# yahoo0742/COSNet

Hardware: AMD Instinct MI355X
Metric: frame-pairs/sec (fwd+bwd) at 473x473 RGBD (higher is better)
Workload: dtype bf16; 1 GPU; RGBDSegmentation_RAA train step (fwd+loss+bwd+SGD), 473x473, batch 4 pairs/GPU; model=RGBDSegmentation_RAA(Bottleneck,[3,4,23,3],[3,4,6,3],1), global_batch=4, parallelism=dp1

## Files before the change

### cosnet_amd/_native.py

```python
import ctypes
import os

import torch

_HERE = os.path.dirname(os.path.abspath(__file__))
LIB_PATH = os.environ.get("COSNET_HIP_LIB") or os.path.join(_HERE, "_lib", "libcosnet_hip.so")

DT_F32 = 0
DT_BF16 = 1

_P = ctypes.c_void_p
_I = ctypes.c_int
_L = ctypes.c_longlong
_F = ctypes.c_float
_S = ctypes.c_size_t

_SIGS = {
    "cn_conv_fwd": (_I, [_I, _P, _L, _I, _I, _I, _I, _P, _I, _I, _I, _I, _I, _I, _P, _P, _L, _I, _I, _P]),
    "cn_conv_fwd_ws": (_I, [_I, _P, _L, _I, _I, _I, _I, _P, _I, _I, _I, _I, _I, _I, _P, _P, _L, _I, _I,
                            _P, _S, _P]),
    "cn_conv_fwd_workspace_floats": (_S, [_I, _I, _I, _I]),
    "cn_conv_dgrad": (_I, [_I, _P, _L, _I, _I, _I, _I, _P, _I, _I, _I, _I, _I, _I, _P, _L, _I, _I, _I, _P]),
    "cn_conv_wgrad_workspace_floats": (_S, [_I, _I, _I, _I, _I, _I, _I, _I]),
    "cn_conv_wgrad": (_I, [_I, _P, _L, _I, _I, _I, _I, _P, _L, _I, _I, _I, _I, _I, _I, _I, _I, _P, _P, _P]),
    "cn_conv_wgrad_grouped": (_I, [_I, _I, _P, _L, _I, _I, _I, _I, _P, _L, _I, _I, _I, _I, _I, _I, _I, _I,
                                   _P, _P]),
    "cn_conv_wgrad_grouped_workspace_floats": (_S, [_I, _I, _I, _I, _I, _I, _I, _I, _I]),
    "cn_conv_wgrad_grouped_ws": (_I, [_I, _I, _P, _L, _I, _I, _I, _I, _P, _L, _I, _I, _I, _I, _I, _I, _I,
                                      _I, _P, _P, _S, _P]),
    "cn_splitk_reduce": (_I, [_P, _I, _L, _L, _P, _I, _P]),
    "cn_fp8_quant": (_I, [_I, _P, _L, _I, _I, _P, _L, _P, _I, _P]),
    "cn_fp8_quant_fmt": (_I, [_I, _I, _P, _L, _I, _I, _P, _L, _P, _I, _P]),
    "cn_conv_dgrad_fp8": (_I, [_P, _L, _I, _I, _I, _I, _P, _I, _I, _I, _I, _I, _P, _L, _I, _I, _I,
                               _P, _P, _P]),
    "cn_fp8_update": (_I, [_P, _I, _F, _P]),
    "cn_fp8_quant_multi": (_I, [_P, _I, _P]),
    "cn_conv_fwd_fp8": (_I, [_P, _L, _I, _I, _I, _I, _P, _I, _I, _I, _I, _I, _I, _P, _P, _L, _I, _I, _P,
                             _P, _P]),
    "cn_conv_fwd_bn_workspace_floats": (_S, [_I, _I, _I, _I]),
    "cn_conv_fwd_bn_grouped": (_I, [_I, _P, _L, _I, _I, _I, _I, _I, _P, _I, _I, _I, _P, _P, _P, _L, _I,
                                    _P, _P, _P, _P, _P, _F, _F, _P]),
    "cn_conv_fwd_fp8_bn": (_I, [_P, _L, _I, _I, _I, _I, _P, _I, _I, _I, _I, _I, _I, _P, _P, _L, _I, _I,
                                _P, _P, _I, _P, _P, _P, _P, _P, _F, _F, _P]),
    "cn_conv_fwd_bn": (_I, [_I, _P, _L, _I, _I, _I, _I, _P, _I, _I, _I, _I, _I, _I, _P, _P, _L, _I, _I,
                            _I, _P, _P, _P, _P, _P, _F, _F, _P]),
    "cn_conv_dgrad_bn_workspace_floats": (_S, [_I, _I, _I, _I]),
    "cn_conv_dgrad_bn": (_I, [_I, _P, _L, _I, _I, _I, _I, _P, _I, _I, _I, _I, _I, _P, _L, _I, _I, _P,
                              _L, _P, _P, _P, _P, _P, _P, _P, _P]),
    "cn_bn_bwd_apply": (_I, [_I, _P, _L, _P, _L, _I, _I, _P, _P, _P, _P, _P, _P, _P, _L, _P]),
    "cn_gemm": (_I, [_I, _I, _I, _I, _I, _I, _I, _I, _P, _L, _L, _P, _L, _L, _P, _L, _L, _I, _I, _F, _P, _I, _I, _L, _P]),
    "cn_bn_workspace_floats": (_S, [_I, _I, _I, _I]),
    "cn_bn_stats": (_I, [_I, _P, _L, _I, _I, _I, _P, _P, _P, _P, _F, _F, _P, _P]),
    "cn_bn_eval_params": (_I, [_P, _P, _I, _F, _P, _P, _P]),
    "cn_bn_apply": (_I, [_I, _P, _L, _I, _I, _I, _P, _P, _P, _P, _P, _L, _P, _L, _P, _P, _P, _P, _I, _P, _P, _L, _P]),
    "cn_bn_apply_fp8": (_I, [_I, _P, _L, _I, _I, _I, _P, _P, _P, _P, _P, _L, _P, _L, _P, _P, _P, _P, _I, _P,
                             _P, _L, _P, _L, _P, _P]),
    "cn_bn_apply_ex": (_I, [_I, _P, _L, _I, _I, _I, _P, _P, _P, _P, _P, _L, _P, _L, _P, _P, _P, _P, _I, _P,
                            _P, _L, _P, _L, _P, _P, _L, _P]),
    "cn_bn_set_tuning": (_I, [_I, _I]),
    "cn_bn_bwd": (_I, [_I, _P, _L, _P, _L, _P, _L, _I, _I, _P, _P, _P, _P, _I, _P, _P, _P, _P, _P, _L, _P, _L, _P, _P]),
    "cn_coatt_workspace_floats": (_S, [_I, _I, _I]),
    "cn_coatt_softmax": (_I, [_I, _P, _I, _I, _I, _P, _P, _P, _P]),
    "cn_coatt_dscore": (_I, [_I, _P, _P, _P, _P, _P, _P, _I, _I, _I, _P, _P]),
    "cn_coatt_fused_fwd": (_I, [_P, _L, _P, _L, _P, _L, _I, _I, _I, _P, _P, _L, _P]),
    "cn_coatt_fused_fwd_ws": (_I, [_P, _L, _P, _L, _P, _L, _I, _I, _I, _P, _P, _L, _P, _S, _P]),
    "cn_coatt_fused_workspace_bytes": (_S, [_I, _I, _I]),
    "cn_coatt_f8_workspace_bytes": (_S, [_I, _I]),
    "cn_coatt_f8_fwd": (_I, [_P, _L, _P, _L, _P, _L, _I, _I, _I, _P, _P, _L, _P, _P, _P, _S, _P]),
    "cn_coatt_f8_train_workspace_bytes": (_S, [_I, _I]),
    "cn_coatt_f8_train_fwd": (_I, [_P, _L, _P, _L, _P, _L, _I, _I, _I, _P, _P, _L, _P, _P, _P, _P, _P, _L, _P, _S, _P]),
    "cn_coatt_flash_fwd": (_I, [_P, _L, _P, _L, _P, _L, _I, _I, _I, _P, _P, _L, _P, _P, _P]),
    "cn_coatt_flash_fwd_ws": (_I, [_P, _L, _P, _L, _P, _L, _I, _I, _I, _P, _P, _L, _P, _P, _P, _S, _P]),
    "cn_coatt_flash_pv": (_I, [_P, _L, _P, _L, _P, _L, _P, _I, _I, _I, _P, _L, _I, _P]),
    "cn_coatt_flash_dvat": (_I, [_P, _L, _P, _L, _P, _L, _P, _L, _P, _L, _P, _P, _P, _P, _I, _I, _I, _P,
                                 _L, _I, _P]),
    "cn_coatt_flash_dvat_ws": (_I, [_P, _L, _P, _L, _P, _L, _P, _L, _P, _L, _P, _P, _P, _P, _I, _I, _I, _P,
                                    _L, _I, _P, _S, _P]),
    "cn_coatt_flash_bwd_workspace_bytes": (_S, [_I, _I]),
    "cn_coatt_flash_pv_ws": (_I, [_P, _L, _P, _L, _P, _L, _P, _I, _I, _I, _P, _L, _I, _P, _S, _P]),
    "cn_rowdot_seg": (_I, [_I, _P, _L, _P, _L, _I, _I, _I, _I, _P, _P]),
    "cn_nchw_to_nhwc": (_I, [_I, _P, _I, _I, _I, _I, _I, _P, _P]),
    "cn_weight_prep": (_I, [_I, _P, _I, _I, _I, _I, _P, _P, _P]),
    "cn_maxpool_fwd": (_I, [_I, _P, _I, _I, _I, _I, _I, _I, _I, _I, _I, _P, _P, _P]),
    "cn_maxpool_bwd": (_I, [_I, _P, _P, _I, _I, _I, _I, _I, _I, _I, _I, _I, _P, _P]),
    "cn_avgpool": (_I, [_I, _P, _L, _I, _I, _I, _F, _P, _P, _P]),
    "cn_avgpool_workspace_floats": (_S, [_I, _I, _I, _I]),
    "cn_bcast_rows": (_I, [_I, _P, _I, _I, _I, _F, _P, _L, _I, _P]),
    "cn_gate_fwd": (_I, [_I, _P, _L, _I, _I, _P, _P, _P, _L, _P, _P]),
    "cn_gate_bwd": (_I, [_I, _P, _L, _P, _L, _P, _I, _I, _P, _I, _P, _L, _P, _P, _P, _P]),
    "cn_colpart_workspace_floats": (_S, [_I, _I]),
    "cn_mean_rows": (_I, [_P, _I, _I, _P, _P]),
    "cn_sum_rows": (_I, [_P, _I, _I, _P, _P]),
    "cn_scale_dev": (_I, [_P, _L, _P, _P, _P]),
    "cn_scale": (_I, [_P, _L, _F, _P]),
    "cn_soft_iou": (_I, [_P, _P, _I, _L, _P, _P, _P, _P]),
    "cn_frame_resize": (_I, [_I, _P, _I, _L, _L, _L, _I, _I, _I, _I, _P, _P, _I, _I, _I, _I, _P]),
    "cn_gemm_force_config": (_I, [_I]),
    "cn_gemm_set_wgrad_target": (_I, [_I]),
    "cn_coatt_force_variant": (_I, [_I]),
    "cn_head_fwd": (_I, [_I, _P, _L, _P, _L, _I, _I, _I, _P, _P, _P, _L, _P, _P]),
    "cn_head_bwd": (_I, [_I, _P, _L, _P, _I, _I, _I, _P, _P, _L, _P, _P, _P, _P]),
    "cn_upsample_sigmoid": (_I, [_P, _I, _I, _I, _I, _I, _I, _P, _P]),
    "cn_upsample_sigmoid_bwd": (_I, [_P, _P, _I, _I, _I, _I, _I, _I, _P, _P]),
    "cn_count_ge": (_I, [_P, _L, _F, _P, _P]),
    "cn_loss_workspace_floats": (_S, [_L]),
    "cn_bce_l1": (_I, [_P, _P, _L, _F, _F, _P, _P, _P, _P]),
    "cn_bce_l1_devcount": (_I, [_P, _P, _L, _P, ctypes.c_double, _F, _P, _P, _P, _P]),
    "cn_sgd": (_I, [_P, _I, _P, _F, _F, _P]),
    "cn_rowdot": (_I, [_I, _P, _L, _P, _L, _I, _I, _P, _P]),
    "cn_colsum": (_I, [_I, _P, _L, _I, _I, _P, _P, _P]),
    "cn_cast2d": (_I, [_I, _I, _P, _L, _I, _I, _P, _L, _I, _P]),
    "cn_build_source_hash": (ctypes.c_char_p, []),
    "cn_build_experimental": (_I, []),
    "cn_conv_wgrad_fp8_workspace_floats": (_S, [_I, _I, _I, _I, _I, _I, _I, _I]),
    "cn_conv_wgrad_fp8": (_I, [_I, _P, _L, _I, _I, _I, _I, _P, _L, _I, _I, _I, _I, _I, _I, _I, _I,
                               _P, _P, _P, _P, _S, _P]),
}

_lib = None


class NativeError(RuntimeError):
    pass


def load():
    global _lib
    if _lib is not None:
        return _lib
    if not os.path.exists(LIB_PATH):
        raise NativeError("libcosnet_hip.so not built (%s); run __graft_entry__.build()" % LIB_PATH)
    lib = ctypes.CDLL(LIB_PATH, mode=ctypes.RTLD_GLOBAL)
    for name, (res, args) in _SIGS.items():
        if os.environ.get("COSNET_HIP_LIB") and not hasattr(lib, name):
            continue
        fn = getattr(lib, name)
        fn.restype = res
        fn.argtypes = args
    _lib = lib
    return lib


HASHED_SOURCES = ["gemm.hip", "conv.hip", "bn.hip", "ew.hip", "coatt.hip", "coatt_fused.hip",
                  "coatt_q48.hip", "coatt_flash.hip", "coatt_f8.hip", "fp8.hip", "frames.hip", "eval.hip",
                  "common.h", "gemm.h", "coatt_fused.h", "../../include/cosnet_hip.h"]


def source_hash():
    import hashlib
    h = hashlib.sha256()
    for f in HASHED_SOURCES:
        with open(os.path.join(_HERE, "csrc", f), "rb") as fh:
            h.update(fh.read())
    return h.hexdigest()[:16]


def build_info():
    import hashlib
    lib_hash = load().cn_build_source_hash().decode()
    with open(LIB_PATH, "rb") as fh:
        so = hashlib.sha256(fh.read()).hexdigest()[:16]
    src = source_hash()
    return {"lib_source_hash": lib_hash, "tree_source_hash": src, "built_from_tree": lib_hash == src,
            "lib_sha256": so, "lib": os.path.relpath(LIB_PATH, os.path.dirname(_HERE))}


def exported_symbols():
    return sorted(_SIGS.keys())


_ERR = {-1: "shape", -2: "alignment", -3: "unsupported", -4: "hip runtime"}


def call(name, *args):
    rc = getattr(load(), name)(*args)
    if rc != 0:
        raise NativeError("%s failed: %s (%d)" % (name, _ERR.get(rc, "hipError"), rc))
    return rc


def query(name, *args):
    return getattr(load(), name)(*args)


def stream():
    return torch.cuda.current_stream().cuda_stream


def ptr(t):
    return None if t is None else t.data_ptr()


def dtype_code(dt):
    if dt == torch.bfloat16:
        return DT_BF16
    if dt == torch.float32:
        return DT_F32
    raise NativeError("unsupported compute dtype %s" % dt)
```

### cosnet_amd/csrc/gemm.h

```cpp
#pragma once
#include "common.h"

enum LoadKind { L_KC_DENSE = 0, L_KC_CONV = 1, L_MC_DENSE = 2, L_MC_CONV = 3,
                L_KC_CONV_G = 4 };

struct ConvGeom {
  int N, H, W, C;
  int OH, OW;
  int KH, KW;
  int st;
  int off_y, off_x, step_y, step_x;
  FastDiv div_C, div_KW, div_OW, div_OHW;
};

constexpr int GEMM_MAXG = 24;
struct GemmGroup {
  const void* A[GEMM_MAXG];
  const void* B[GEMM_MAXG];
  void* C[GEMM_MAXG];
  const float* SA[GEMM_MAXG];
  const float* SB[GEMM_MAXG];
  const float* bias[GEMM_MAXG];
  float* ST[GEMM_MAXG];
  int dil[GEMM_MAXG];
};

struct GemmArgs {
  int M, N, K;
  int ka_lim, kb_lim;
  const void* A; long long lda, a_bs;
  const void* B; long long ldb, b_bs;
  void* C; long long ldc, c_bs;
  const float* bias;
  ConvGeom ga, gb;
  int k_chunk, nsplit;
  int row_map;
  FastDiv rm_div_OW, rm_div_OHW;
  int rm_H, rm_W;
  int c_mode;
  long long slab;
  float alpha;
  const float* scale_a;
  const float* scale_b;
  int cfg;
  int st_mode;
  float* st_ws;
  long long st_plane;
  int st_seg_rows;
  const void* br_x; long long br_ldx;
  const float* br_mean; const float* br_invstd; const float* br_gamma; const float* br_beta;
  int ngroup;
  GemmGroup grp;
  int wt;
};

int cn_gemm_dispatch(const GemmArgs& a, int dtype, int c_f32, int la, int lb, int batch, hipStream_t st);
int cn_gemm_pick(int M, int N, int K, int batch_splits);
long long cn_gemm_cfg_blocks(int cfg, int M, int N);
int cn_gemm_bm(int dtype, int M, int N, int K, int cfg_or_minus1);
int cn_splitk_reduce_impl(const float* ws, int nsplit, long long slab, long long n, float* out,
                          int accumulate, hipStream_t st);
```

### cosnet_amd/csrc/gemm.hip

```cpp
#include "common.h"
#include "gemm.h"
#include "../../include/cosnet_hip.h"

#include <cstdlib>
#include <type_traits>

namespace {

template <class T> struct Frag;
template <> struct Frag<bf16> { typedef bf16x8 type; };
template <> struct Frag<float> { typedef f32x4 type; };

__device__ __forceinline__ int mc_swz(int k, int granules_per_row) {
  int h = (k & 3) | (((k >> 3) & 1) << 2);
  return (granules_per_row >= 32 ? h : (h & 3)) << 2;
}

__device__ __forceinline__ int mc_swz8(int k) { return (k & 7) ^ ((k >> 5) & 1); }

__device__ __attribute__((aligned(16))) unsigned g_zero16[4];

__device__ __forceinline__ void glds16(const void* src, char* lds_wave_base) {
  __builtin_amdgcn_global_load_lds((const __attribute__((address_space(1))) void*)src,
                                   (__attribute__((address_space(3))) void*)lds_wave_base, 16, 0, 0);
}

constexpr unsigned BUF_OOB = 0x80000000u;
__device__ __forceinline__ __amdgpu_buffer_rsrc_t buf_rsrc(const void* base) {
  return __builtin_amdgcn_make_buffer_rsrc(const_cast<void*>(base), 0, (int)BUF_OOB, 0x00020000);
}
__device__ __forceinline__ void blds16(__amdgpu_buffer_rsrc_t r, unsigned voff, unsigned soff,
                                       char* lds_wave_base) {
  __builtin_amdgcn_raw_ptr_buffer_load_lds(r, (__attribute__((address_space(3))) void*)lds_wave_base,
                                           16, (int)voff, (int)soff, 0, 0);
}

template <class T, int ROWS, int KIND, int NT> struct Loader {
  static constexpr int VEC = VecOf<T>::N;
  static constexpr int BK = 8 * VEC;
  static constexpr int NCH = ROWS * 8 / NT;
  static constexpr int RSTEP = NT / 8;
  static_assert(NCH >= 1 && NCH * NT == ROWS * 8, "tile rows must fill whole chunk rounds");
  static constexpr bool MC = (KIND == L_MC_DENSE || KIND == L_MC_CONV);
  static constexpr bool BUF = (KIND == L_KC_DENSE || KIND == L_KC_CONV || KIND == L_MC_DENSE);
  static constexpr int CPR = ROWS / VEC;
  static constexpr int KROW_STEP = NT / CPR;
  static constexpr int RB = ROWS * (int)sizeof(T);
  static constexpr unsigned SZ = sizeof(T);
  static_assert(!(MC && sizeof(T) == 1) || CPR == 8, "fp8 MC tiles are 128 columns wide (mc_swz8)");

  long long ld;
  int klim;
  int kbeg;
  int kcol;
  bool ok[NCH];
  __amdgpu_buffer_rsrc_t rsrc;
  unsigned voff[NCH];
  int img[NCH], by[NCH], bx[NCH];
  int ctap;
  const T* base;
  const T* ptr[NCH];
  int ry[NCH], sx[NCH], cic[NCH];
  int pim[NCH], poy[NCH], pox[NCH], pp[NCH];
  int ax, ay, aim;
  ConvGeom g;

  __device__ __forceinline__ void init(const T* b, long long ld_, int lim, int klim_,
                                       const ConvGeom& geo, int origin, int tid, int kbeg_) {
    ld = ld_; klim = klim_; kbeg = kbeg_;
    base = b;
    if (!MC) {
      const int pos = tid & 7;
      kcol = (pos ^ ((tid >> 3) & 7)) * VEC;
      if (KIND == L_KC_DENSE) rsrc = buf_rsrc(b + (long long)origin * ld);
      if (KIND == L_KC_CONV) rsrc = buf_rsrc(b);
#pragma unroll
      for (int i = 0; i < NCH; ++i) {
        const int rl = (tid >> 3) + RSTEP * i;
        const int row = origin + rl;
        ok[i] = row < lim;
        const int rr = ok[i] ? row : 0;
        if (KIND == L_KC_DENSE) {
          voff[i] = ok[i] ? (unsigned)((rl * ld + kcol) * SZ) : BUF_OOB;
        } else {
          int q, rem, oy, ox;
          fdivmod(rr, geo.div_OHW, q, rem);
          fdivmod(rem, geo.div_OW, oy, ox);
          img[i] = ok[i] ? q : -1;
          by[i] = oy * geo.st + geo.off_y;
          bx[i] = ox * geo.st + geo.off_x;
        }
      }
      if (KIND == L_KC_CONV || KIND == L_KC_CONV_G) {
        g = geo;
        ctap = -1;
      }
    } else {
      const int pos = tid % CPR;
      if (KIND == L_MC_DENSE) rsrc = buf_rsrc(b + (long long)kbeg_ * ld + origin);
#pragma unroll
      for (int i = 0; i < NCH; ++i) {
        const int krl = tid / CPR + KROW_STEP * i;
        const int cchunk = (sizeof(T) == 2) ? (pos ^ (mc_swz(krl, RB / 8) >> 1))
                         : (sizeof(T) == 1) ? (pos ^ mc_swz8(krl)) : pos;
        const int col = origin + cchunk * VEC;
        ok[i] = col < lim;
        if (KIND == L_MC_DENSE) {
          voff[i] = ok[i] ? (unsigned)((krl * ld + cchunk * VEC) * SZ) : BUF_OOB;
        } else {
          const int nn = ok[i] ? col : 0;
          int tap, r, s2;
          fdivmod(nn, geo.div_C, tap, cic[i]);
          fdivmod(tap, geo.div_KW, r, s2);
          ry[i] = r * geo.step_y + geo.off_y;
          sx[i] = s2 * geo.step_x + geo.off_x;
          pp[i] = kbeg_ + krl;
          int q, rem, oy, ox;
// ... 104 lines not shown
    }
  }
};

template <int ROWS, bool MC>
__device__ __forceinline__ bf16x8 read_frag_bf16(const char* lds, int rowbase, int p, int lane) {
  int g = lane >> 4;
  if (!MC) {
    int row = rowbase + (lane & 15);
    int c = 4 * p + g;
    return *(const bf16x8*)(lds + row * 128 + ((c ^ (row & 7)) << 4));
  } else {
    constexpr int RB = ROWS * 2;
    int q = (lane & 15) >> 2, pp = lane & 3;
    int gm = (rowbase >> 2) + pp;
    int k1 = 32 * p + 8 * g + q, k2 = k1 + 4;
    const char* a1 = lds + k1 * RB + ((gm ^ mc_swz(k1, RB / 8)) << 3);
    const char* a2 = lds + k2 * RB + ((gm ^ mc_swz(k2, RB / 8)) << 3);
    s16x4 lo = __builtin_amdgcn_ds_read_tr16_b64_v4i16(LDS_PTR(s16x4, a1));
    s16x4 hi = __builtin_amdgcn_ds_read_tr16_b64_v4i16(LDS_PTR(s16x4, a2));
    typedef __attribute__((ext_vector_type(8))) short s16x8;
    s16x8 r = __builtin_shufflevector(lo, hi, 0, 1, 2, 3, 4, 5, 6, 7);
    return __builtin_bit_cast(bf16x8, r);
  }
}

__device__ __forceinline__ i32x8 read_frag_f8(const char* lds, int rowbase, int lane) {
  const int row = rowbase + (lane & 15), g = lane >> 4;
  const u32x4 lo = *(const u32x4*)(lds + row * 128 + (((2 * g) ^ (row & 7)) << 4));
  const u32x4 hi = *(const u32x4*)(lds + row * 128 + (((2 * g + 1) ^ (row & 7)) << 4));
  i32x8 r;
  r[0] = lo.x; r[1] = lo.y; r[2] = lo.z; r[3] = lo.w; r[4] = hi.x; r[5] = hi.y; r[6] = hi.z; r[7] = hi.w;
  return r;
}

typedef __attribute__((ext_vector_type(2))) int i32x2;
__device__ __forceinline__ i32x8 read_frag_f8_mc(const char* lds, int colbase, int lane) {
  const int i = lane & 15, g = lane >> 4, q = i >> 1, pp = i & 1;
  const int cb = colbase >> 4;
  i32x8 r;
#pragma unroll
  for (int j = 0; j < 4; ++j) {
    const int k = 32 * g + 8 * j + q;
    const char* a = lds + k * 128 + ((cb ^ mc_swz8(k)) << 4) + 8 * pp;
    const i32x2 v = __builtin_amdgcn_ds_read_tr8_b64_v2i32(LDS_PTR(i32x2, a));
    r[2 * j] = v.x;
    r[2 * j + 1] = v.y;
  }
  return r;
}

template <int ROWS>
__device__ __forceinline__ f32x4 read_frag_f32_kc(const char* lds, int rowbase, int p, int lane) {
  int row = rowbase + (lane & 15);
  int c = 4 * p + (lane >> 4);
  return *(const f32x4*)(lds + row * 128 + ((c ^ (row & 7)) << 4));
}
template <int ROWS>
__device__ __forceinline__ float read_frag_f32_mc(const char* lds, int rowbase, int p, int j, int lane) {
  int k = 16 * p + 4 * (lane >> 4) + j;
  int col = rowbase + (lane & 15);
  return *(const float*)(lds + k * (ROWS * 4) + col * 4);
}

template <class CT> __device__ __forceinline__ void store_c(CT* c, float v, int mode);
template <> __device__ __forceinline__ void store_c<float>(float* c, float v, int mode) {
  if (mode == 1) atomicAdd(c, v);
  else if (mode == 2) *c += v;
  else *c = v;
}
template <> __device__ __forceinline__ void store_c<bf16>(bf16* c, float v, int mode) {
  if (mode == 2) v += (float)*c;
  *c = (bf16)v;
}

}

template <int G>
__device__ __forceinline__ void wait_tiles(int n) {
  if (n <= 0) asm volatile("s_waitcnt vmcnt(0)" ::: "memory");
  else if (n == 1) asm volatile("s_waitcnt vmcnt(%0)" :: "n"(G) : "memory");
  else if (n == 2) asm volatile("s_waitcnt vmcnt(%0)" :: "n"(2 * G) : "memory");
  else asm volatile("s_waitcnt vmcnt(%0)" :: "n"(3 * G) : "memory");
}

__device__ __forceinline__ void raw_barrier() {
  asm volatile("" ::: "memory");
  __builtin_amdgcn_s_barrier();
  asm volatile("" ::: "memory");
}

#ifndef CN_GEMM_GROUP_M
#define CN_GEMM_GROUP_M 8
#endif
#ifndef CN_GEMM_PRIO
#define CN_GEMM_PRIO 0
#endif
#ifndef CN_GEMM_ZREMAP
#define CN_GEMM_ZREMAP 1
#endif

template <class T, class CT, int BM, int BN, int WM, int WN, int S, int LA, int LB, int EPI = 0, int PP = 0>
__global__ __launch_bounds__(WM * WN * 64 * (PP == 2 ? 2 : 1), (EPI && sizeof(T) == 2 && BM * BN <= 128 * 128 && S == 2) ? 4 : 1) void gemm_kernel(GemmArgs p) {
  constexpr bool KSG = PP == 2;
  constexpr int NT = WM * WN * 64 * (KSG ? 2 : 1);
  constexpr int VEC = VecOf<T>::N;
  constexpr int BK = 8 * VEC;
  constexpr int ABYTES = BM * 128, BBYTES = BN * 128;
  constexpr int STAGE = ABYTES + BBYTES;
  constexpr int TM = BM / WM, TN = BN / WN;
  constexpr int RM = TM / 16, RN = TN / 16;
  constexpr bool AMC = (LA == L_MC_DENSE || LA == L_MC_CONV);
  constexpr bool BMC = (LB == L_MC_DENSE || LB == L_MC_CONV);
  typedef Loader<T, BM, LA, NT> LdA;
  typedef Loader<T, BN, LB, NT> LdB;
  constexpr int G = LdA::NCH + LdB::NCH;
  static_assert(S >= 2 && S <= 4, "2..4 stages");
  __shared__ __attribute__((aligned(16))) char smem[S * STAGE];

  const int tid = threadIdx.x, lane = tid & 63, wave = tid >> 6;
  const int kg = KSG ? wave / (WM * WN) : 0;
  const int wl = KSG ? wave % (WM * WN) : wave;
  const int wm = wl / WN, wn = wl % WN;
  static_assert(!KSG || (sizeof(T) == 2 && !AMC && !BMC), "KSG: bf16 k-contiguous operands");
  int tm, tn, bz;
  {
    const int nwg = gridDim.x * gridDim.y;
#if CN_GEMM_ZREMAP
    const int all = nwg * gridDim.z;
    const int orig = blockIdx.x + blockIdx.y * gridDim.x + blockIdx.z * nwg;
#else
    const int all = nwg;
    const int orig = blockIdx.x + blockIdx.y * gridDim.x;
#endif
    int glin = orig;
    if (all >= 16) {
      const int xcd = orig & 7, q = all >> 3, r = all & 7;
      glin = (xcd < r ? xcd * (q + 1) : r * (q + 1) + (xcd - r) * q) + (orig >> 3);
    }
#if CN_GEMM_ZREMAP
    bz = glin / nwg;
#else
    bz = blockIdx.z;
#endif
    const int lin = glin - (glin / nwg) * nwg;
#if CN_GEMM_GROUP_M > 0
    {
      const int gm = CN_GEMM_GROUP_M;
      const int per = gm * gridDim.y;
      const int grp = lin / per, first = grp * gm;
      const int gsz = min((int)gridDim.x - first, gm);
      const int r = lin - grp * per;
      tm = first + r % gsz;
      tn = r / gsz;
    }
#else
    tm = lin % gridDim.x;
    tn = lin / gridDim.x;
#endif
  }
  const int m0 = tm * BM, n0 = tn * BN;
  const int batch = bz / p.nsplit, split = bz - batch * p.nsplit;
  int kbeg = split * p.k_chunk;
  int kend = min(p.K, kbeg + p.k_chunk);
  ConvGeom gA = p.ga;
  if constexpr (LA == L_KC_CONV) {
    if (p.ngroup && p.grp.dil[batch] > 0) {
      const int dl = p.grp.dil[batch];
      gA.off_y = gA.off_x = -dl;
      gA.step_y = gA.step_x = dl;
    }
  }
// ... 653 lines not shown
          const int c = pick_cfg(a, batch);
          if (c == 18) return launch_c<T, CT, 18, LA, LB>(a, batch, st);
          if (c == 19) return launch_c<T, CT, 19, LA, LB>(a, batch, st);
          return launch_c<T, CT, 20, LA, LB>(a, batch, st);
        } else {
          if (pick_cfg(a, batch) == 20) return launch_c<T, CT, 10, LA, LB>(a, batch, st);
          return launch_c<T, CT, 11, LA, LB>(a, batch, st);
        }
      }
      default: return launch_c<T, CT, 12, LA, LB>(a, batch, st);
    }
  }
}

template <class T, class CT>
static int launch_conv_g(const GemmArgs& a, int batch, hipStream_t st) {
  if constexpr (sizeof(T) == 4) {
    if (a.N <= 64 || cfg_blocks(1, a, batch) < 384) return launch_c<T, CT, 0, L_KC_CONV_G, L_KC_DENSE>(a, batch, st);
    return launch_c<T, CT, 1, L_KC_CONV_G, L_KC_DENSE>(a, batch, st);
  } else {
    const int c = pick_cfg(a, batch);
    if (c == 12) return launch_c<T, CT, 12, L_KC_CONV_G, L_KC_DENSE>(a, batch, st);
    if (c == 13) return launch_c<T, CT, 13, L_KC_CONV_G, L_KC_DENSE>(a, batch, st);
    return launch_c<T, CT, 11, L_KC_CONV_G, L_KC_DENSE>(a, batch, st);
  }
}

template <class T, class CT>
static int launch_kinds(const GemmArgs& a, int la, int lb, int batch, hipStream_t st) {
#define CN_CASE(A_, B_) \
  if (la == A_ && lb == B_) return launch_tile<T, CT, A_, B_>(a, batch, st);
  if (la == L_KC_CONV_G && lb == L_KC_DENSE) return launch_conv_g<T, CT>(a, batch, st);
  CN_CASE(L_KC_DENSE, L_KC_DENSE)
  CN_CASE(L_KC_CONV, L_KC_DENSE)
  CN_CASE(L_KC_DENSE, L_MC_DENSE)
  CN_CASE(L_MC_DENSE, L_MC_DENSE)
  CN_CASE(L_MC_DENSE, L_MC_CONV)
#undef CN_CASE
  return -10;
}

template <class CT, int LA, class T8 = f8e4m3>
static int launch_f8(const GemmArgs& a, int batch, hipStream_t st) {
  static const int big = [] { const char* e = getenv("CN_GEMM_F8BIG"); return e ? atoi(e) : 0; }();
  const int c = pick_cfg(a, batch);
  if constexpr (sizeof(CT) == 2 && std::is_same<T8, f8e4m3>::value) {
    if (a.st_mode == 1) {
      if (c == 12) return launch_c<T8, CT, 12, LA, L_KC_DENSE, 1>(a, batch, st);
      if (c == 13) return launch_c<T8, CT, 13, LA, L_KC_DENSE, 1>(a, batch, st);
      return launch_c<T8, CT, 11, LA, L_KC_DENSE, 1>(a, batch, st);
    }
  }
  if (a.st_mode) return CN_ERR_UNSUPPORTED;
  if ((big == 8 || big == 9) && c != 12 && tiles_of(big, a.M, a.N) * batch >= 256) {
    if (big == 8) return launch_c<T8, CT, 8, LA, L_KC_DENSE>(a, batch, st);
    return launch_c<T8, CT, 9, LA, L_KC_DENSE>(a, batch, st);
  }
  if (c == 12) return launch_c<T8, CT, 12, LA, L_KC_DENSE>(a, batch, st);
  if (c == 13) return launch_c<T8, CT, 13, LA, L_KC_DENSE>(a, batch, st);
  return launch_c<T8, CT, 11, LA, L_KC_DENSE>(a, batch, st);
}

template <int LB>
static int launch_f8_mc(const GemmArgs& a, int batch, hipStream_t st) {
  if (a.cfg == 13) return launch_c<f8e5m2, float, 13, L_MC_DENSE, LB>(a, batch, st);
  return launch_c<f8e5m2, float, 11, L_MC_DENSE, LB>(a, batch, st);
}

static bool buf_ok(int kind, const GemmArgs& a, bool is_a, int esz) {
  const long long ld = is_a ? a.lda : a.ldb;
  const ConvGeom& g = is_a ? a.ga : a.gb;
  const long long kspan = a.nsplit > 1 ? a.k_chunk : a.K;
  if (kind == L_KC_DENSE) return 256 * ld * esz < 0x80000000ll && (long long)a.K * esz < 0xFFFF0000ll;
  if (kind == L_KC_CONV) return (long long)g.N * g.H * g.W * ld * esz < 0x80000000ll;
  if (kind == L_MC_DENSE) return (kspan + 128) * ld * esz < 0xFFFF0000ll && 128 * ld * esz < 0x80000000ll;
  return true;
}

static int wt_on() {
  static const int lvl = [] { const char* e = getenv("CN_GEMM_WT"); return e ? atoi(e) : 4; }();
  return lvl;
}

int cn_gemm_dispatch(const GemmArgs& a_in, int dtype, int c_f32, int la, int lb, int batch, hipStream_t st) {
  GemmArgs a = a_in;
  a.wt = wt_on() == 4 ? (a.c_mode != 1 && a.c_mode != 3 ? 4 : 0)
                      : !a.row_map && a.c_mode != 1 && (wt_on() == 1 || (wt_on() == 3 && a.c_mode == 3));
  if (a.M <= 0 || a.N <= 0 || batch <= 0) return 0;
  const int esz = (dtype == DT_FP8 || dtype == DT_FP8_E5M2) ? 1 : dtype == DT_BF16 ? 2 : 4;
  const int bk = 128 / esz;
  if (la == L_KC_CONV && (a.ga.C % bk != 0 || !buf_ok(L_KC_CONV, a, true, esz))) la = L_KC_CONV_G;
  if (!buf_ok(la, a, true, esz) || !buf_ok(lb, a, false, esz)) return CN_ERR_SHAPE;
  if (dtype == DT_FP8) {
    if (lb != L_KC_DENSE || a.nsplit != 1) return CN_ERR_UNSUPPORTED;
    if (a.st_mode && (a.st_mode != 1 || batch != 1 || a.row_map || a.c_mode || c_f32)) return CN_ERR_UNSUPPORTED;
    if (la == L_KC_DENSE) return c_f32 ? launch_f8<float, L_KC_DENSE>(a, batch, st) : launch_f8<bf16, L_KC_DENSE>(a, batch, st);
    if (la == L_KC_CONV) return c_f32 ? launch_f8<float, L_KC_CONV>(a, batch, st) : launch_f8<bf16, L_KC_CONV>(a, batch, st);
    if (la == L_KC_CONV_G) return c_f32 ? launch_f8<float, L_KC_CONV_G>(a, batch, st) : launch_f8<bf16, L_KC_CONV_G>(a, batch, st);
    return CN_ERR_UNSUPPORTED;
  }
  if (dtype == DT_FP8_E5M2 && la == L_MC_DENSE) {
    if (!c_f32 || a.st_mode || a.row_map || a.c_mode == 1 || a.c_mode == 2) return CN_ERR_UNSUPPORTED;
    if (lb == L_MC_DENSE) return launch_f8_mc<L_MC_DENSE>(a, batch, st);
    if (lb == L_MC_CONV) return launch_f8_mc<L_MC_CONV>(a, batch, st);
    return CN_ERR_UNSUPPORTED;
  }
  if (dtype == DT_FP8_E5M2) {
    if (lb != L_KC_DENSE || a.st_mode || a.nsplit != 1 || c_f32) return CN_ERR_UNSUPPORTED;
    if (la == L_KC_DENSE) return launch_f8<bf16, L_KC_DENSE, f8e5m2>(a, batch, st);
    if (la == L_KC_CONV) return launch_f8<bf16, L_KC_CONV, f8e5m2>(a, batch, st);
    if (la == L_KC_CONV_G) return launch_f8<bf16, L_KC_CONV_G, f8e5m2>(a, batch, st);
    return CN_ERR_UNSUPPORTED;
  }
  if (a.st_mode) {
    if ((batch != 1 && !(a.ngroup == batch && a.st_mode == 1)) || a.nsplit != 1 || a.row_map || a.c_mode ||
        lb != L_KC_DENSE || (la != L_KC_DENSE && la != L_KC_CONV && la != L_KC_CONV_G))
      return CN_ERR_UNSUPPORTED;
#define CN_EPI(T_, M_) \
    return la == L_KC_DENSE ? launch_epi<T_, L_KC_DENSE, M_>(a, batch, st) : \
           la == L_KC_CONV ? launch_epi<T_, L_KC_CONV, M_>(a, batch, st) : launch_epi<T_, L_KC_CONV_G, M_>(a, batch, st)
    if (dtype == DT_BF16) {
      if (a.st_mode == 1) CN_EPI(bf16, 1); else CN_EPI(bf16, 2);
    } else {
      if (a.st_mode == 1) CN_EPI(float, 1); else CN_EPI(float, 2);
    }
#undef CN_EPI
  }
  if (dtype == DT_BF16) {
    return c_f32 ? launch_kinds<bf16, float>(a, la, lb, batch, st)
                 : launch_kinds<bf16, bf16>(a, la, lb, batch, st);
  } else if (dtype == DT_F32) {
    return launch_kinds<float, float>(a, la, lb, batch, st);
  }
  return -11;
}

int cn_gemm_bm(int dtype, int M, int N, int K, int cfg) {
  if (dtype != DT_BF16) return kCfg[1].bm;
  if (g_force_cfg >= 0 && g_force_cfg < kNumCfg) return kCfg[g_force_cfg].bm;
  if (cfg >= 0 && cfg < kNumCfg) return kCfg[cfg].bm;
  return kCfg[heuristic_cfg(M, N, K, 1)].bm;
}

int cn_gemm_pick(int M, int N, int K, int batch_splits) {
  if (g_force_cfg >= 0 && g_force_cfg < kNumCfg) return g_force_cfg;
  return heuristic_cfg(M, N, K, batch_splits);
}

long long cn_gemm_cfg_blocks(int cfg, int M, int N) {
  GemmArgs a = {};
  a.M = M; a.N = N; a.nsplit = 1;
  return cfg_blocks(cfg, a, 1);
}

extern "C" int cn_gemm_force_config(int cfg) {
  if (cfg >= kNumCfg || (!CN_EXPERIMENTAL && cfg >= 21)) return -1;
  g_force_cfg = cfg;
  return kNumCfg;
}

template <int G>
__global__ __launch_bounds__(256) void splitk_reduce_k(const float* __restrict__ ws, int nsplit,
                                                       long long slab, long long n4,
                                                       float* __restrict__ out, int accumulate) {
  constexpr int OPB = 256 / G;
  __shared__ f32x4 red[G][OPB];
  const int o = threadIdx.x % OPB, g = threadIdx.x / OPB;
  for (long long base = (long long)blockIdx.x * OPB; base < n4; base += (long long)gridDim.x * OPB) {
    const long long i = base + o;
    f32x4 a = {0.f, 0.f, 0.f, 0.f};
    if (i < n4) {
      int s = g;
      for (; s + 7 * G < nsplit; s += 8 * G) {
        f32x4 v[8];
#pragma unroll
        for (int u = 0; u < 8; ++u) v[u] = *(const f32x4*)(ws + (long long)(s + u * G) * slab + 4 * i);
#pragma unroll
        for (int u = 0; u < 8; ++u) a += v[u];
      }
      for (; s < nsplit; s += G) a += *(const f32x4*)(ws + (long long)s * slab + 4 * i);
    }
    if (G > 1) {
      red[g][o] = a;
      __syncthreads();
      if (g == 0) {
#pragma unroll
        for (int q = 1; q < G; ++q) a += red[q][o];
      }
      __syncthreads();
    }
    if (g == 0 && i < n4) {
      if (accumulate) a += ((const f32x4*)out)[i];
      ((f32x4*)out)[i] = a;
    }
  }
}

int cn_splitk_reduce_impl(const float* ws, int nsplit, long long slab, long long n, float* out,
                          int accumulate, hipStream_t st) {
  if (n % 4 || slab % 4) return -2;
  const long long n4 = n / 4;
  int G = 1;
  while (G < 16 && 2 * G <= nsplit && n4 * G < (512ll << 10)) G *= 2;
  const int opb = 256 / G;
  long long b = (n4 + opb - 1) / opb;
  if (b > 4096) b = 4096;
#define CN_RED(GG) \
  hipLaunchKernelGGL(splitk_reduce_k<GG>, dim3((unsigned)b), dim3(256), 0, st, ws, nsplit, slab, n4, out, accumulate)
  switch (G) {
    case 1: CN_RED(1); break;
    case 2: CN_RED(2); break;
    case 4: CN_RED(4); break;
    case 8: CN_RED(8); break;
    default: CN_RED(16); break;
  }
#undef CN_RED
  CN_CHECK_LAUNCH();
  return 0;
}
```

### include/cosnet_hip.h

```cpp
#ifndef COSNET_HIP_H
#define COSNET_HIP_H
#include <stddef.h>
#include <hip/hip_runtime_api.h>

#ifdef __cplusplus
extern "C" {
#endif

#define CN_ERR_SHAPE (-1)
#define CN_ERR_ALIGN (-2)
#define CN_ERR_UNSUPPORTED (-3)
#define CN_ERR_HIP (-4)


int cn_conv_fwd(int dtype, const void* x, long long ldx, int N, int H, int W, int Cin,
                const void* w, int Cout, int KH, int KW, int stride, int pad, int dil,
                const float* bias, void* y, long long ldy, int OH, int OW, hipStream_t stream);

size_t cn_conv_fwd_workspace_floats(int dtype, int M, int Cout, int K);
int cn_conv_fwd_ws(int dtype, const void* x, long long ldx, int N, int H, int W, int Cin,
                   const void* w, int Cout, int KH, int KW, int stride, int pad, int dil,
                   const float* bias, void* y, long long ldy, int OH, int OW, float* ws,
                   size_t ws_floats, hipStream_t stream);

// ... 140 lines not shown
                          hipStream_t st);
int cn_coatt_flash_pv(const void* q, long long ldq, const void* k, long long ldk, const void* v,
                      long long ldv, const float* klse, int B, int HW, int C, void* o, long long ldo,
                      int accumulate, hipStream_t stream);
int cn_coatt_flash_pv_ws(const void* q, long long ldq, const void* k, long long ldk, const void* v,
                         long long ldv, const float* klse, int B, int HW, int C, void* o,
                         long long ldo, int accumulate, void* ws, size_t ws_bytes, hipStream_t stream);

int cn_coatt_flash_dvat(const void* vat, long long ld_vat, const void* va, long long ld_va,
                        const void* dza, long long ld_dza, const void* vb, long long ld_vb,
                        const void* dzb, long long ld_dzb, const float* lse_a, const float* d0,
                        const float* lse_b, const float* d1, int B, int HW, int C, void* out,
                        long long ld_out, int accumulate, hipStream_t stream);
size_t cn_coatt_flash_bwd_workspace_bytes(int B, int HW);
int cn_coatt_flash_dvat_ws(const void* vat, long long ld_vat, const void* va, long long ld_va,
                           const void* dza, long long ld_dza, const void* vb, long long ld_vb,
                           const void* dzb, long long ld_dzb, const float* lse_a, const float* d0,
                           const float* lse_b, const float* d1, int B, int HW, int C, void* out,
                           long long ld_out, int accumulate, void* ws, size_t ws_bytes,
                           hipStream_t stream);

int cn_nchw_to_nhwc(int dtype, const float* x, int N, int C, int H, int W, int Cp, void* y,
                    hipStream_t stream);
int cn_weight_prep(int dtype, const float* w, int Cout, int KHW, int Cin, int Cp, void* wf,
                   void* wt, hipStream_t stream);
int cn_maxpool_fwd(int dtype, const void* x, int N, int H, int W, int C, int OH, int OW, int k,
                   int s, int pad, void* y, unsigned char* argmax, hipStream_t stream);
int cn_maxpool_bwd(int dtype, const void* dy, const unsigned char* argmax, int N, int H, int W,
                   int C, int OH, int OW, int k, int s, int pad, void* dx, hipStream_t stream);
int cn_avgpool(int dtype, const void* x, long long ld, int N, int HW, int C, float scale, void* y,
               float* ws , hipStream_t stream);
size_t cn_avgpool_workspace_floats(int dtype, int N, int HW, int C);
int cn_bcast_rows(int dtype, const void* src, int N, int HW, int C, float scale, void* dst,
                  long long ld, int accumulate, hipStream_t stream);
int cn_gate_fwd(int dtype, const void* z, long long ldz, int P, int C, const float* g,
                const float* gb, void* out, long long ldo, float* mask, hipStream_t stream);
int cn_gate_bwd(int dtype, const void* z, long long ldz, const void* dout, long long lddo,
                const float* mask, int P, int C, const float* g, int through_mask, void* dz,
                long long lddz, float* dg, float* dgb,
                float* ws , hipStream_t stream);
int cn_mean_rows(const float* x, int nrows, int C, float* out, hipStream_t stream);
int cn_sum_rows(const float* x, int nrows, int C, float* out, hipStream_t stream);
int cn_scale(float* x, long long n, float s, hipStream_t stream);
int cn_scale_dev(const float* x, long long n, const float* s, float* out, hipStream_t stream);
int cn_soft_iou(const float* x, const unsigned char* gt, int nframes, long long hw,
                unsigned char* mask, double* iou, long long* counts, hipStream_t stream);
size_t cn_colpart_workspace_floats(int P, int C);
int cn_head_fwd(int dtype, const void* a, long long lda, const void* b, long long ldb, int P,
                int C, int relu, const float* w, const float* bias, void* zout, long long ldz,
                float* logit, hipStream_t stream);
int cn_head_bwd(int dtype, const void* z, long long ldz, const float* dlogit, int P, int C,
                int relu, const float* w, void* dz, long long lddz, float* dw, float* db,
                float* ws , hipStream_t stream);
int cn_upsample_sigmoid(const float* in, int N, int h, int w, int H, int W, int apply_sigmoid,
                        float* out, hipStream_t stream);
int cn_upsample_sigmoid_bwd(const float* dout, const float* out, int N, int h, int w, int H,
                            int W, int apply_sigmoid, float* din, hipStream_t stream);
int cn_count_ge(const float* gt, long long n, float thr, unsigned long long* cnt,
                hipStream_t stream);
size_t cn_loss_workspace_floats(long long n);
int cn_bce_l1(const float* pred, const float* gt, long long n, float weight, float l1w, float* ws,
              float* loss, float* dpred, hipStream_t stream);
int cn_bce_l1_devcount(const float* pred, const float* gt, long long n, const long long* pos_count,
                       double total, float l1w, float* ws, float* loss, float* dpred,
                       hipStream_t stream);
int cn_sgd(const void* tensors, int nt, const float* lrs, float wd, float momentum,
           hipStream_t stream);
int cn_rowdot(int dtype, const void* a, long long lda, const void* b, long long ldb, int P, int C,
              float* out, hipStream_t stream);
int cn_rowdot_seg(int dtype, const void* a, long long lda, const void* b, long long ldb, int P, int C,
                  int seg, int seg_ld, float* out, hipStream_t stream);
int cn_colsum(int dtype, const void* x, long long ld, int P, int C, float* out,
              float* ws , hipStream_t stream);
int cn_cast2d(int dtype_in, int dtype_out, const void* x, long long ldx, int P, int C, void* y,
              long long ldy, int accumulate, hipStream_t stream);
int cn_frame_resize(int src_u8, const void* src, int C, long long plane_stride, long long row_stride,
                    long long col_stride, int y0, int x0, int h, int w, const float* mean,
                    float* dst, int H, int W, int mode, int flip, hipStream_t stream);

const char* cn_build_source_hash(void);
int cn_build_experimental(void);

int cn_gemm_force_config(int cfg);
int cn_gemm_set_wgrad_target(int blocks);
int cn_coatt_force_variant(int v);

#ifdef __cplusplus
}
#endif
#endif
```

Before: 132.3 frame-pairs/s.

## Add persistent weight-stationary GEMM for small-K bf16 dense matmuls

Adds a new persistent GEMM kernel for bf16 dense GEMMs with small K (64 to 512) and large M. It keeps the B (weight) slice resident in LDS and registers while each workgroup walks a contiguous range of M rows, with XCD-aware walker assignment. A tiles are double-buffered and residual C is prefetched for accumulate mode. It targets the 1x1 convolutions in the ResNet bottlenecks and is enabled by default through a heuristic (K<=256, N>=4K, M>=8192). The risk is lower parallelism, since only one block per CU per slice is used, and a new code path that may be slower than the tuned generic kernels.

```diff
diff --git a/cosnet_amd/_native.py b/cosnet_amd/_native.py
--- a/cosnet_amd/_native.py
+++ b/cosnet_amd/_native.py
@@ -96,6 +96,8 @@
     "cn_soft_iou": (_I, [_P, _P, _I, _L, _P, _P, _P, _P]),
     "cn_frame_resize": (_I, [_I, _P, _I, _L, _L, _L, _I, _I, _I, _I, _P, _P, _I, _I, _I, _I, _P]),
     "cn_gemm_force_config": (_I, [_I]),
+    "cn_gemm_ws_mode": (_I, [_I]),
+    "cn_gemm_ws_launches": (_S, []),
     "cn_gemm_set_wgrad_target": (_I, [_I]),
     "cn_coatt_force_variant": (_I, [_I]),
     "cn_head_fwd": (_I, [_I, _P, _L, _P, _L, _I, _I, _I, _P, _P, _P, _L, _P, _P]),
@@ -141,9 +143,9 @@
     return lib
 
 
-HASHED_SOURCES = ["gemm.hip", "conv.hip", "bn.hip", "ew.hip", "coatt.hip", "coatt_fused.hip",
+HASHED_SOURCES = ["gemm.hip", "gemm_ws.hip", "conv.hip", "bn.hip", "ew.hip", "coatt.hip", "coatt_fused.hip",
                   "coatt_q48.hip", "coatt_flash.hip", "coatt_f8.hip", "fp8.hip", "frames.hip", "eval.hip",
-                  "common.h", "gemm.h", "coatt_fused.h", "../../include/cosnet_hip.h"]
+                  "common.h", "gemm.h", "gemm_dev.h", "coatt_fused.h", "../../include/cosnet_hip.h"]
 
 
 def source_hash():
diff --git a/cosnet_amd/csrc/gemm.h b/cosnet_amd/csrc/gemm.h
--- a/cosnet_amd/csrc/gemm.h
+++ b/cosnet_amd/csrc/gemm.h
@@ -58,5 +58,7 @@
 int cn_gemm_pick(int M, int N, int K, int batch_splits);
 long long cn_gemm_cfg_blocks(int cfg, int M, int N);
 int cn_gemm_bm(int dtype, int M, int N, int K, int cfg_or_minus1);
+bool cn_gemm_ws_supports(const GemmArgs& a);
+int cn_gemm_ws_launch(const GemmArgs& a, int walkers_per_xcd, hipStream_t st);
 int cn_splitk_reduce_impl(const float* ws, int nsplit, long long slab, long long n, float* out,
                           int accumulate, hipStream_t st);
diff --git a/cosnet_amd/csrc/gemm.hip b/cosnet_amd/csrc/gemm.hip
--- a/cosnet_amd/csrc/gemm.hip
+++ b/cosnet_amd/csrc/gemm.hip
@@ -1,5 +1,6 @@
 #include "common.h"
 #include "gemm.h"
+#include "gemm_dev.h"
 #include "../../include/cosnet_hip.h"
 
 #include <cstdlib>
@@ -23,16 +24,6 @@
 __device__ __forceinline__ void glds16(const void* src, char* lds_wave_base) {
   __builtin_amdgcn_global_load_lds((const __attribute__((address_space(1))) void*)src,
                                    (__attribute__((address_space(3))) void*)lds_wave_base, 16, 0, 0);
-}
-
-constexpr unsigned BUF_OOB = 0x80000000u;
-__device__ __forceinline__ __amdgpu_buffer_rsrc_t buf_rsrc(const void* base) {
-  return __builtin_amdgcn_make_buffer_rsrc(const_cast<void*>(base), 0, (int)BUF_OOB, 0x00020000);
-}
-__device__ __forceinline__ void blds16(__amdgpu_buffer_rsrc_t r, unsigned voff, unsigned soff,
-                                       char* lds_wave_base) {
-  __builtin_amdgcn_raw_ptr_buffer_load_lds(r, (__attribute__((address_space(3))) void*)lds_wave_base,
-                                           16, (int)voff, (int)soff, 0, 0);
 }
 
 template <class T, int ROWS, int KIND, int NT> struct Loader {
@@ -303,12 +294,6 @@
   else if (n == 1) asm volatile("s_waitcnt vmcnt(%0)" :: "n"(G) : "memory");
   else if (n == 2) asm volatile("s_waitcnt vmcnt(%0)" :: "n"(2 * G) : "memory");
   else asm volatile("s_waitcnt vmcnt(%0)" :: "n"(3 * G) : "memory");
-}
-
-__device__ __forceinline__ void raw_barrier() {
-  asm volatile("" ::: "memory");
-  __builtin_amdgcn_s_barrier();
-  asm volatile("" ::: "memory");
 }
 
 #ifndef CN_GEMM_GROUP_M
@@ -1128,6 +1113,28 @@
   return lvl;
 }
 
+static int g_ws_mode = -1;
+static size_t g_ws_launches = 0;
+static int ws_mode() {
+  if (g_ws_mode < 0) {
+    const char* e = getenv("CN_GEMM_WS");
+    const int v = e ? atoi(e) : 1;
+    g_ws_mode = (v >= 0 && v <= 3) ? v : 1;
+  }
+  return g_ws_mode;
+}
+static bool ws_heuristic(const GemmArgs& a) {
+  return a.K <= 256 && a.N >= 4 * a.K && a.M >= 8192;
+}
+static bool ws_eligible(const GemmArgs& a, int dtype, int c_f32, int la, int lb, int batch) {
+  if (!ws_mode() || g_force_cfg >= 0 || a.cfg >= 0) return false;
+  if (dtype != DT_BF16 || c_f32 || la != L_KC_DENSE || lb != L_KC_DENSE) return false;
+  if (batch != 1 || a.nsplit != 1 || a.row_map || a.ngroup || a.st_mode) return false;
+  if ((a.c_mode != 0 && a.c_mode != 2) || a.bias || a.alpha != 1.f || a.scale_a || a.scale_b) return false;
+  if (!cn_gemm_ws_supports(a)) return false;
+  return ws_mode() >= 2 || ws_heuristic(a);
+}
+
 int cn_gemm_dispatch(const GemmArgs& a_in, int dtype, int c_f32, int la, int lb, int batch, hipStream_t st) {
   GemmArgs a = a_in;
   a.wt = wt_on() == 4 ? (a.c_mode != 1 && a.c_mode != 3 ? 4 : 0)
@@ -1137,6 +1144,10 @@
   const int bk = 128 / esz;
   if (la == L_KC_CONV && (a.ga.C % bk != 0 || !buf_ok(L_KC_CONV, a, true, esz))) la = L_KC_CONV_G;
   if (!buf_ok(la, a, true, esz) || !buf_ok(lb, a, false, esz)) return CN_ERR_SHAPE;
+  if (ws_eligible(a, dtype, c_f32, la, lb, batch)) {
+    ++g_ws_launches;
+    return cn_gemm_ws_launch(a, ws_mode() == 3 ? 1 : 0, st);
+  }
   if (dtype == DT_FP8) {
     if (lb != L_KC_DENSE || a.nsplit != 1) return CN_ERR_UNSUPPORTED;
     if (a.st_mode && (a.st_mode != 1 || batch != 1 || a.row_map || a.c_mode || c_f32)) return CN_ERR_UNSUPPORTED;
@@ -1204,6 +1215,15 @@
   g_force_cfg = cfg;
   return kNumCfg;
 }
+
+extern "C" int cn_gemm_ws_mode(int mode) {
+  if (mode < 0 || mode > 3) return -1;
+  const int prev = ws_mode();
+  g_ws_mode = mode;
+  return prev;
+}
+
+extern "C" size_t cn_gemm_ws_launches(void) { return g_ws_launches; }
 
 template <int G>
 __global__ __launch_bounds__(256) void splitk_reduce_k(const float* __restrict__ ws, int nsplit,
diff --git a/cosnet_amd/csrc/gemm_dev.h b/cosnet_amd/csrc/gemm_dev.h
--- /dev/null
+++ b/cosnet_amd/csrc/gemm_dev.h
@@ -0,0 +1,24 @@
+#pragma once
+#include "common.h"
+
+constexpr unsigned BUF_OOB = 0x80000000u;
+__device__ __forceinline__ __amdgpu_buffer_rsrc_t buf_rsrc(const void* base) {
+  return __builtin_amdgcn_make_buffer_rsrc(const_cast<void*>(base), 0, (int)BUF_OOB, 0x00020000);
+}
+__device__ __forceinline__ void blds16(__amdgpu_buffer_rsrc_t r, unsigned voff, unsigned soff,
+                                       char* lds_wave_base) {
+  __builtin_amdgcn_raw_ptr_buffer_load_lds(r, (__attribute__((address_space(3))) void*)lds_wave_base,
+                                           16, (int)voff, (int)soff, 0, 0);
+}
+
+__device__ __forceinline__ void raw_barrier() {
+  asm volatile("" ::: "memory");
+  __builtin_amdgcn_s_barrier();
+  asm volatile("" ::: "memory");
+}
+
+__device__ __forceinline__ bf16x8 read_frag_kc_bf16(const char* lds, int rowbase, int p, int lane) {
+  const int row = rowbase + (lane & 15);
+  const int c = 4 * p + (lane >> 4);
+  return *(const bf16x8*)(lds + row * 128 + ((c ^ (row & 7)) << 4));
+}
diff --git a/cosnet_amd/csrc/gemm_ws.hip b/cosnet_amd/csrc/gemm_ws.hip
--- /dev/null
+++ b/cosnet_amd/csrc/gemm_ws.hip
@@ -0,0 +1,260 @@
+#include "common.h"
+#include "gemm.h"
+#include "gemm_dev.h"
+#include "../../include/cosnet_hip.h"
+
+#include <algorithm>
+#include <cstdlib>
+#include <type_traits>
+
+namespace {
+
+struct WsArgs {
+  int M, N;
+  const bf16* A; long long lda;
+  const bf16* B; long long ldb;
+  bf16* C; long long ldc;
+  int nslices;
+  int wpx;
+  int wt;
+};
+
+__device__ __forceinline__ u32x4 load16_asm(const void* p) {
+  u32x4 v;
+  asm volatile("global_load_dwordx4 %0, %1, off" : "=&v"(v) : "v"(p) : "memory");
+  return v;
+}
+
+template <int KEEP, bool TIE, int N>
+__device__ __forceinline__ void wait_keep(u32x4 (&x)[N]) {
+  static_assert(KEEP < 64, "vmcnt is 6 bits");
+  asm volatile("s_waitcnt vmcnt(%0)" :: "n"(KEEP) : "memory");
+  if constexpr (TIE) {
+#pragma unroll
+    for (int i = 0; i < N; ++i) asm volatile("" : "+v"(x[i]));
+  }
+}
+
+template <int KT, int BM, int BN, int WM, int WN, bool MODE2, bool BREG>
+__global__ __launch_bounds__(WM * WN * 64, 1) void gemm_ws_kernel(WsArgs p) {
+  constexpr int NT = WM * WN * 64;
+  constexpr int BBYTES = KT * BN * 128, ASTG = KT * BM * 128;
+  constexpr int TM = BM / WM, TN = BN / WN;
+  constexpr int RM = TM / 16, RN = TN / 16;
+  constexpr int NCA = BM * 8 / NT, NCB = BN * 8 / NT;
+  constexpr int RSTEP = NT / 8;
+  constexpr int CSB = TM * TN * 4;
+  constexpr int GPR = TN / 8, RPP = 64 / GPR, IT = TM / RPP;
+  static_assert(NCA >= 1 && NCA * NT == BM * 8 && NCB * NT == BN * 8, "tiles fill whole chunk rounds");
+  static_assert(RSTEP % 8 == 0, "a thread's chunks share row & 7");
+  static_assert(IT >= 1 && IT * RPP == TM && (RN & (RN - 1)) == 0, "epilogue passes");
+  static_assert(BBYTES + 2 * ASTG + WM * WN * CSB <= 160 * 1024, "LDS budget");
+  __shared__ __attribute__((aligned(16))) char smem[BBYTES + 2 * ASTG + WM * WN * CSB];
+
+  const int tid = threadIdx.x, lane = tid & 63;
+  const int wave = __builtin_amdgcn_readfirstlane(tid >> 6);
+  const int wm = wave / WN, wn = wave % WN;
+
+  const int xcd = blockIdx.x & 7, j = blockIdx.x >> 3;
+  const int slice = j % p.nslices;
+  const int walker = xcd * p.wpx + j / p.nslices, nwalk = 8 * p.wpx;
+  const int n0 = slice * BN;
+  const int m16 = (p.M + 15) >> 4;
+  const int r0 = (int)((long long)m16 * walker / nwalk) * 16;
+  const int r1 = min(p.M, (int)((long long)m16 * (walker + 1) / nwalk) * 16);
+  if (r0 >= r1) return;
+  const int ntiles = (r1 - r0 + BM - 1) / BM;
+
+  char* Bs = smem;
+  char* As = smem + BBYTES;
+  float* cs = (float*)(smem + BBYTES + 2 * ASTG + wave * CSB);
+  const int wbase = __builtin_amdgcn_readfirstlane((tid & ~63) * 16);
+
+  const int kcol = ((tid & 7) ^ ((tid >> 3) & 7)) * 8;
+  const int rl0 = tid >> 3;
+
+  {
+    const __amdgpu_buffer_rsrc_t rb = buf_rsrc(p.B + (long long)n0 * p.ldb);
+#pragma unroll
+    for (int i = 0; i < NCB; ++i) {
+      const int rl = rl0 + RSTEP * i;
+      const unsigned voff = n0 + rl < p.N ? (unsigned)((rl * p.ldb + kcol) * 2) : BUF_OOB;
+#pragma unroll
+      for (int kt = 0; kt < KT; ++kt) blds16(rb, voff, kt * 128, Bs + kt * BN * 128 + wbase + i * NT * 16);
+    }
+  }
+  auto issue_a = [&](int t, char* stg) {
+    const int m0 = r0 + t * BM;
+    const __amdgpu_buffer_rsrc_t ra = buf_rsrc(p.A + (long long)m0 * p.lda);
+#pragma unroll
+    for (int i = 0; i < NCA; ++i) {
+      const int rl = rl0 + RSTEP * i;
+      const unsigned voff = m0 + rl < r1 ? (unsigned)((rl * p.lda + kcol) * 2) : BUF_OOB;
+#pragma unroll
+      for (int kt = 0; kt < KT; ++kt) blds16(ra, voff, kt * 128, stg + kt * BM * 128 + wbase + i * NT * 16);
+    }
+  };
+  const int erow = wm * TM + lane / GPR, ecol = n0 + wn * TN + (lane % GPR) * 8;
+  const bool col_ok = ecol < p.N;
+  u32x4 xnx[MODE2 ? IT : 1], xpf[MODE2 ? IT : 1];
+  auto fetch_c = [&](int t) {
+    const int m0 = r0 + t * BM;
+#pragma unroll
+    for (int it = 0; it < IT; ++it) {
+      const int row = m0 + erow + it * RPP;
+      const bf16* src = (row < r1 && col_ok) ? p.C + (long long)row * p.ldc + ecol : p.C;
+      xnx[it] = load16_asm(src);
+    }
+  };
+  issue_a(0, As);
+  if constexpr (MODE2) fetch_c(0);
+  wait_keep<0, MODE2>(xnx);
+  raw_barrier();
+
+  bf16x8 breg[BREG ? KT * 2 : 1][RN];
+  if constexpr (BREG) {
+#pragma unroll
+    for (int kt = 0; kt < KT; ++kt)
+#pragma unroll
+      for (int pc = 0; pc < 2; ++pc)
+#pragma unroll
+        for (int jj = 0; jj < RN; ++jj)
+          breg[kt * 2 + pc][jj] = read_frag_kc_bf16(Bs + kt * BN * 128, wn * TN + jj * 16, pc, lane);
+  }
+
+  auto epilogue = [&](int t, auto aux_c, const f32x4 (&acc)[RM][RN]) {
+    constexpr int AUX = decltype(aux_c)::value;
+    const int m0 = r0 + t * BM;
+    const __amdgpu_buffer_rsrc_t rc = buf_rsrc(p.C + (long long)m0 * p.ldc);
+    const int g = lane >> 4;
+#pragma unroll
+    for (int i = 0; i < RM; ++i)
+#pragma unroll
+      for (int jj = 0; jj < RN; ++jj)
+#pragma unroll
+        for (int r = 0; r < 4; ++r)
+          cs[(i * 16 + 4 * g + r) * TN + (((jj ^ (g & (RN - 1))) << 4) | (lane & 15))] = acc[i][jj][r];
+    asm volatile("s_waitcnt lgkmcnt(0)" ::: "memory");
+#pragma unroll
+    for (int it = 0; it < IT; ++it) {
+      const int rr = lane / GPR + it * RPP;
+      const int c0 = ((lane % GPR) * 8) ^ ((((rr >> 2) & 3) & (RN - 1)) << 4);
+      float v[8];
+      *(f32x4*)&v[0] = *(const f32x4*)&cs[rr * TN + c0];
+      *(f32x4*)&v[4] = *(const f32x4*)&cs[rr * TN + c0 + 4];
+      if constexpr (MODE2) {
+        float q[8];
+        Chunk<bf16>::unpack(xpf[it], q);
+#pragma unroll
+        for (int e = 0; e < 8; ++e) v[e] += q[e];
+      }
+      const int row = erow + it * RPP;
+      const unsigned off = (m0 + row < r1 && col_ok) ? (unsigned)(((long long)row * p.ldc + ecol) * 2) : BUF_OOB;
+      __builtin_amdgcn_raw_buffer_store_b128(Chunk<bf16>::pack(v), rc, (int)off, 0, AUX);
+    }
+    asm volatile("" ::: "memory");
+  };
+
+#pragma unroll 1
+  for (int t = 0; t < ntiles; ++t) {
+    char* cur = As + (t & 1) * ASTG;
+    if constexpr (MODE2) {
+#pragma unroll
+      for (int it = 0; it < IT; ++it) xpf[it] = xnx[it];
+    }
+    if (t + 1 < ntiles) {
+      issue_a(t + 1, As + ((t + 1) & 1) * ASTG);
+      if constexpr (MODE2) fetch_c(t + 1);
+    }
+    f32x4 acc[RM][RN];
+#pragma unroll
+    for (int i = 0; i < RM; ++i)
+#pragma unroll
+      for (int jj = 0; jj < RN; ++jj) acc[i][jj] = (f32x4){0.f, 0.f, 0.f, 0.f};
+#pragma unroll
+    for (int kt = 0; kt < KT; ++kt)
+#pragma unroll
+      for (int pc = 0; pc < 2; ++pc) {
+        bf16x8 af[RM], bfr[RN];
+#pragma unroll
+        for (int i = 0; i < RM; ++i) af[i] = read_frag_kc_bf16(cur + kt * BM * 128, wm * TM + i * 16, pc, lane);
+#pragma unroll
+        for (int jj = 0; jj < RN; ++jj) {
+          if constexpr (BREG) bfr[jj] = breg[kt * 2 + pc][jj];
+          else bfr[jj] = read_frag_kc_bf16(Bs + kt * BN * 128, wn * TN + jj * 16, pc, lane);
+        }
+#pragma unroll
+        for (int i = 0; i < RM; ++i)
+#pragma unroll
+          for (int jj = 0; jj < RN; ++jj)
+            acc[i][jj] = __builtin_amdgcn_mfma_f32_16x16x32_bf16(af[i], bfr[jj], acc[i][jj], 0, 0, 0);
+      }
+    if (p.wt == 4) epilogue(t, std::integral_constant<int, 2>{}, acc);
+    else if (p.wt) epilogue(t, std::integral_constant<int, 16>{}, acc);
+    else epilogue(t, std::integral_constant<int, 0>{}, acc);
+    if (t + 1 < ntiles) {
+      wait_keep<IT, MODE2>(xnx);
+      raw_barrier();
+    }
+  }
+}
+
+template <int KT, int BM, int BN, int WM, int WN, bool BREG>
+int launch_ws(const GemmArgs& a, int cus, int cap, hipStream_t st) {
+  WsArgs w;
+  w.M = a.M; w.N = a.N;
+  w.A = (const bf16*)a.A; w.lda = a.lda;
+  w.B = (const bf16*)a.B; w.ldb = a.ldb;
+  w.C = (bf16*)a.C; w.ldc = a.ldc;
+  w.nslices = (a.N + BN - 1) / BN;
+  w.wt = a.wt;
+  const int per_xcd = cus / 8;
+  const int want = (int)((((long long)a.M + 15) / 16 + 7) / 8);
+  w.wpx = std::min(per_xcd / w.nslices, std::max(want, 1));
+  if (cap > 0) w.wpx = std::min(w.wpx, cap);
+  if (w.wpx < 1) return CN_ERR_UNSUPPORTED;
+  const dim3 grid(8 * w.wpx * w.nslices), block(WM * WN * 64);
+  if (a.c_mode == 2)
+    hipLaunchKernelGGL((gemm_ws_kernel<KT, BM, BN, WM, WN, true, BREG>), grid, block, 0, st, w);
+  else
+    hipLaunchKernelGGL((gemm_ws_kernel<KT, BM, BN, WM, WN, false, BREG>), grid, block, 0, st, w);
+  CN_CHECK_LAUNCH();
+  return 0;
+}
+
+int device_cus() {
+  static const int n = [] {
+    int dev = 0, v = 0;
+    if (hipGetDevice(&dev) != hipSuccess) return 0;
+    if (hipDeviceGetAttribute(&v, hipDeviceAttributeMultiprocessorCount, dev) != hipSuccess) return 0;
+    return v;
+  }();
+  return n;
+}
+
+int ws_bn(int K) { return K == 512 ? 64 : 128; }
+
+}
+
+bool cn_gemm_ws_supports(const GemmArgs& a) {
+  if (a.K != 64 && a.K != 128 && a.K != 256 && a.K != 512) return false;
+  if (a.ka_lim < a.K || a.kb_lim < a.K) return false;
+  if (a.N % 8 || a.ldc % 8 || (uintptr_t)a.C % 16) return false;
+  if (a.lda % 8 || a.ldb % 8 || (uintptr_t)a.A % 16 || (uintptr_t)a.B % 16) return false;
+  if (256 * a.ldc * 2 >= 0x80000000ll) return false;
+  const int cus = device_cus();
+  return cus >= 8 && (a.N + ws_bn(a.K) - 1) / ws_bn(a.K) <= cus / 8;
+}
+
+int cn_gemm_ws_launch(const GemmArgs& a, int walkers_per_xcd, hipStream_t st) {
+  const int cus = device_cus();
+  switch (a.K) {
+    case 64:
+      if (a.c_mode == 2) return launch_ws<1, 64, 128, 2, 2, true>(a, cus, walkers_per_xcd, st);
+      return launch_ws<1, 128, 128, 4, 2, true>(a, cus, walkers_per_xcd, st);
+    case 128: return launch_ws<2, 128, 128, 4, 2, true>(a, cus, walkers_per_xcd, st);
+    case 256: return launch_ws<4, 64, 128, 2, 4, true>(a, cus, walkers_per_xcd, st);
+    case 512: return launch_ws<8, 32, 64, 2, 2, false>(a, cus, walkers_per_xcd, st);
+    default: return CN_ERR_UNSUPPORTED;
+  }
+}
diff --git a/include/cosnet_hip.h b/include/cosnet_hip.h
--- a/include/cosnet_hip.h
+++ b/include/cosnet_hip.h
@@ -246,6 +246,8 @@
 int cn_build_experimental(void);
 
 int cn_gemm_force_config(int cfg);
+int cn_gemm_ws_mode(int mode);
+size_t cn_gemm_ws_launches(void);
 int cn_gemm_set_wgrad_target(int blocks);
 int cn_coatt_force_variant(int v);
 
```

Result: faster. 134.8 frame-pairs/s, median of 6 (+1.9%).
